# Illumina/strelka

Measured on AMD Instinct MI355X. Metric: candidate-alignment scoring cells/s (read bases x candidate alignments; Strelka2 has no pair-HMM, SURVEY.md section 0) + germline loci/s + 40x WGS-like germline wall-clock (e2e) + 110x/40x somatic wall-clock (e2e_somatic), higher is better.
Workload: dtype f64; 1 GPU; germline chr20-style synthetic (BASELINE.json configs[1]).  Headline: scoreCandidateAlignment as one function -- per GPU per step 65536 reads of 150 bp x 87.9 candidate alignments each (5-7 candidate indels around them), from the candidate alignments the device search left (PCal) to one double each: one kernel (F5: the walk of each alignment's path + the terms of its bases, penalties and clips).  ; read_len=150

## Files before the change

include/strelka_amd.h:

```cpp
#ifndef STRELKA_AMD_H
#define STRELKA_AMD_H

#include <stddef.h>
#include <stdint.h>

#ifdef __cplusplus
extern "C" {
#endif

#define SK_VERSION 100


int sk_device_count(void);
void* sk_host_alloc(size_t bytes);
void sk_host_free(void* p);
int sk_init(int device);
int sk_init_strict(int device);
void sk_shutdown(void);
const char* sk_last_error(void);
int sk_version(void);
int sk_is_initialized(void);
int sk_sync_mode(void);
int sk_libm_restated(void);

int sk_broker_client(void);
int sk_broker_enable(int on);
int sk_broker_serve(int device, const char* socket_name, int idle_seconds);
int sk_broker_selftest(int n, uint32_t mul);

int sk_check_device_errors(void);

int sk_debug_set_g3_variant(int variant);
int sk_debug_g3_global_pass_count(void);
int sk_debug_force_device_libm(int on);
void sk_debug_grown_bytes(int64_t* device_bytes, int64_t* pinned_bytes);
void sk_debug_region_alleles(int no_edge_deletion, int ids_twice);
int sk_debug_f5_tail_order(const int32_t* cal_off, int32_t n_reads, int32_t waves, int32_t shift, int32_t* first, int32_t* n, int32_t* order_out);
int64_t sk_debug_f5_tail_launches(void);

int sk_get_qscore_tables(double* q2p, double* q2lncompe, double* q2lne);


enum { SK_BAM_REF = 0, SK_BAM_A = 1, SK_BAM_C = 2, SK_BAM_G = 4, SK_BAM_T = 8, SK_BAM_ANY = 15 };

enum {
    SK_OP_BASES = 0,
    SK_OP_SOFT_CLIP = 1,
    SK_OP_NOBASE = 2
};
enum { SK_OPFLAG_NONCANDIDATE_PENALTY = 1 };

typedef struct sk_score_op {
    uint16_t length;
// ... 886 lines not shown
```

strelka_amd/capi.py:

```python
import ctypes as C
import os

import numpy as np

_HERE = os.path.dirname(os.path.abspath(__file__))
LIB_PATH = os.path.join(_HERE, "lib", "libstrelka_amd.so")

c_void_p = C.c_void_p


class ScoreOp(C.Structure):
    _fields_ = [("length", C.c_uint16), ("kind", C.c_uint8), ("flags", C.c_uint8), ("src", C.c_int32)]


SCORE_OP_DTYPE = np.dtype([("length", "<u2"), ("kind", "u1"), ("flags", "u1"), ("src", "<i4")])
OP_BASES, OP_SOFT_CLIP, OP_NOBASE = 0, 1, 2
OPFLAG_PENALTY = 1


class AlignBatch(C.Structure):
    _fields_ = [("n_reads", C.c_int32), ("n_cals", C.c_int32), ("n_ops", C.c_int64),
                ("read_off", c_void_p), ("read_code", c_void_p), ("read_qual", c_void_p),
                ("hap_off", c_void_p), ("hap_code", c_void_p), ("cal_off", c_void_p), ("op_off", c_void_p),
                ("ops", c_void_p), ("max_read_len", C.c_int32), ("max_hap_len", C.c_int32),
# ... 200 lines not shown
    "sk_intake_options_default", "sk_read_intake_obs_bound", "sk_read_intake", "sk_read_intake_dev", "sk_read_intake_scratch_bytes",
    "sk_ar_state_initial", "sk_ref_anchors", "sk_ref_anchors_dev", "sk_active_regions_bound", "sk_active_regions", "sk_active_regions_dev",
    "sk_sync_state_initial", "sk_sync_regions_bound", "sk_sync_active_regions", "sk_sync_active_regions_dev", "sk_sync_region_params", "sk_sync_region_params_dev",
    "sk_region_haplotypes_params", "sk_region_haplotypes_params_dev",
    "sk_region_haplotypes_seq_bound", "sk_region_haplotypes_support_bound", "sk_region_haplotypes_scratch_bytes", "sk_region_haplotypes", "sk_region_haplotypes_dev",
    "sk_region_alleles_allele_bound", "sk_region_alleles_insert_bound", "sk_region_alleles_scratch_bytes", "sk_region_alleles", "sk_region_alleles_dev", "sk_debug_region_alleles",
    "sk_align_builder_create", "sk_align_builder_destroy", "sk_align_builder_clear", "sk_align_builder_append", "sk_align_builder_add_read",
    "sk_align_builder_finish", "sk_align_builder_error", "sk_align_builder_set_host_threads",
    "sk_align_scores_default", "sk_global_align",
    "sk_pileup_options_default", "sk_pileup_reads", "sk_pileup_reads_dev", "sk_pileup_scratch_bytes",
    "sk_pileup_stream_create", "sk_pileup_stream_destroy", "sk_pileup_stream_begin_region", "sk_pileup_stream_push", "sk_pileup_stream_push_begin", "sk_pileup_stream_push_finish", "sk_pileup_stream_enable_evs_words", "sk_gvcf_site_summaries", "sk_gvcf_site_summaries_dev", "sk_gvcf_plain_runs_dev", "sk_gvcf_plain_runs", "sk_pileup_stream_set_gvcf_block_options",
    "sk_somatic_pileup_stream_create", "sk_somatic_pileup_stream_destroy", "sk_somatic_pileup_stream_begin_region", "sk_somatic_pileup_stream_push", "sk_somatic_pileup_stream_push_begin", "sk_somatic_pileup_stream_push_finish",
    "sk_realign_options_default", "sk_realign_job_create", "sk_realign_job_destroy", "sk_realign_job_error",
    "sk_realign_job_set_reference", "sk_realign_job_set_indels", "sk_realign_job_add_read", "sk_realign_job_add_reads", "sk_realign_job_get_batch",
    "sk_realign_job_finish", "sk_realign_job_run", "sk_realign_job_n_reads", "sk_realign_job_read_result",
    "sk_realign_job_clear_reads", "sk_realign_job_rescore", "sk_realign_job_indels_consulted", "sk_realign_job_enumeration_counts", "sk_realign_device_job_counts", "sk_debug_f5_tail_order", "sk_debug_f5_tail_launches", "sk_realign_reference_reads_outside", "sk_realign_job_stage3_counts", "sk_make_start_pos_alignment", "sk_get_end_pin_start_pos",
    "sk_germline_options_default", "sk_dependent_eprob", "sk_dependent_eprob_dev", "sk_site_digt_call",
    "sk_site_digt_call_dev", "sk_site_digt_call_fused", "sk_site_digt_call_fused_dev",
    "sk_somatic_snv_options_default", "sk_somatic_snv_call_batch", "sk_somatic_snv_call_batch_dev",
    "sk_somatic_snv_call_tiers", "sk_somatic_snv_call_tiers_dev", "sk_somatic_snv_tiers_scratch_bytes",
    "sk_indel_options_default", "sk_somatic_indel_options_default", "sk_indel_grid_lhood", "sk_indel_grid_lhood_dev",
    "sk_somatic_indel_call_batch", "sk_somatic_indel_call_tiers", "sk_allele_group_genotype_lhoods", "sk_allele_group_genotype_lhoods_dev",
    "sk_allele_group_genotype_lhoods_wide", "sk_allele_group_genotype_lhoods_wide_dev",
    "sk_allele_group_genotype_lhoods_xwide", "sk_allele_group_genotype_lhoods_xwide_dev",
    "sk_discover_indels_and_mismatches", "sk_global_align_scratch_bytes", "sk_global_align_dev", "sk_bai_query", "sk_bam_region_filter", "sk_gvcf_block_sites", "sk_gvcf_block_sites_dev",
]

_lib = None


def lib():
# ... 24 lines not shown
        L.sk_pileup_reads.argtypes = [C.POINTER(ReadBatchStruct), C.POINTER(PileupOptions), C.c_int, C.POINTER(PileupColumns)]
        L.sk_pileup_scratch_bytes.restype = C.c_int64
        L.sk_pileup_scratch_bytes.argtypes = [C.c_int32, C.c_int64, C.c_int32]
        L.sk_pileup_reads_dev.argtypes = [C.POINTER(ReadBatchStruct), C.c_int64, C.POINTER(PileupOptions), C.c_int,
                                          C.POINTER(PileupColumns), c_void_p, c_void_p]
        L.sk_realign_options_default.argtypes = [C.POINTER(RealignOptions)]
        L.sk_realign_job_create.restype = c_void_p
        L.sk_realign_job_create.argtypes = [C.POINTER(RealignOptions)]
        L.sk_realign_job_destroy.argtypes = [c_void_p]
        L.sk_realign_job_enumeration_counts.argtypes = [c_void_p, c_void_p, c_void_p, c_void_p]
        L.sk_realign_device_job_counts.argtypes = [c_void_p, c_void_p, c_void_p]
        L.sk_realign_device_job_counts.restype = None
        L.sk_debug_f5_tail_order.argtypes = [c_void_p, C.c_int32, C.c_int32, C.c_int32, c_void_p, c_void_p, c_void_p]
        L.sk_debug_f5_tail_launches.argtypes = []
        L.sk_debug_f5_tail_launches.restype = C.c_int64
        L.sk_realign_reference_reads_outside.argtypes = []
        L.sk_realign_reference_reads_outside.restype = C.c_int64
        L.sk_realign_job_stage3_counts.argtypes = [c_void_p, c_void_p, c_void_p]
        L.sk_realign_job_indels_consulted.argtypes = [c_void_p, c_void_p, C.c_int32]
        L.sk_realign_job_error.restype = C.c_char_p
        L.sk_realign_job_error.argtypes = [c_void_p]
        L.sk_realign_job_set_reference.argtypes = [c_void_p, C.c_char_p, C.c_int32, C.c_int32]
        L.sk_realign_job_set_indels.argtypes = [c_void_p, C.POINTER(IndelInfo), C.c_int32]
        L.sk_realign_job_add_read.argtypes = [c_void_p, C.POINTER(ReadInput)]
        L.sk_realign_job_add_reads.argtypes = [c_void_p, C.POINTER(ReadInput), C.c_int32]
        L.sk_realign_job_get_batch.argtypes = [c_void_p, C.POINTER(AlignBatch)]
        L.sk_realign_job_finish.argtypes = [c_void_p, c_void_p]
        L.sk_realign_job_run.argtypes = [c_void_p]
        L.sk_realign_job_n_reads.argtypes = [c_void_p]
        L.sk_realign_job_read_result.argtypes = [c_void_p, C.c_int32, C.POINTER(ReadResult)]
# ... 706 lines not shown
        a, b, c = C.c_int64(), C.c_int64(), C.c_int64()
        lib().sk_realign_job_enumeration_counts(self._j, C.byref(a), C.byref(b), C.byref(c))
        return a.value, b.value, c.value

    @staticmethod
    def device_job_counts():
        a, b, c = C.c_int64(), C.c_int64(), C.c_int64()
        lib().sk_realign_device_job_counts(C.byref(a), C.byref(b), C.byref(c))
        return a.value, b.value, c.value

    @staticmethod
    def f5_tail_launches():
        return int(lib().sk_debug_f5_tail_launches())

    @staticmethod
    def f5_tail_order(cal_off, waves, shift):
        cal_off = np.ascontiguousarray(cal_off, np.int32)
        n_reads = len(cal_off) - 1
        first, n = C.c_int32(-1), C.c_int32(-1)
        order = np.full(max(n_reads, 1), -2, np.int32)
        if lib().sk_debug_f5_tail_order(_p(cal_off), n_reads, int(waves), int(shift), C.byref(first), C.byref(n), _p(order)):
            raise StrelkaAmdError(last_error())
        return first.value, order[:n.value].copy()

    def stage3_counts(self):
        a, b = C.c_int64(), C.c_int64()
        lib().sk_realign_job_stage3_counts(self._j, C.byref(a), C.byref(b))
        return a.value, b.value

    def clear_reads(self):
# ... 798 lines not shown
```

strelka_amd/csrc/read_enumerate.hip:

```cpp

#include "sk_common.h"

#include "align_entry.h"
#include "read_enumerate.h"

#include <algorithm>
#include <chrono>
#include <climits>
#include <cstdio>
#include <cstdlib>
#include <cstring>
#include <vector>

using namespace skcore;

int sk_score_alignments_launch_hostleg(const sk_align_batch* b, double* dev_out_lnp, void* hip_stream);

namespace
{

static_assert(sizeof(PFrame) % 4 == 0 && sizeof(PCal) % 4 == 0, "frames move through LDS as 32-bit words");


struct EnumArgs
// ... 235 lines not shown
    a.sorted[a.cal_off[r] + rank] = a.grouped[g];
    }
}


enum { DYN_N_GROUPED = 0, DYN_N_CALS, DYN_N_LIGHT, DYN_N_HEAVY, DYN_FLAGS, DYN_MAX_CALS, DYN_REF_OUTSIDE, DYN_COUNT = 8 };
enum { DYNF_DEEPER = 1,
       DYNF_POOL_FULL = 2 };
enum { SEARCH_LEVELS = Caps::K + 2,
       CNT_LEVELS = 0,
       CNT_LEAVES = Caps::K + 3,
       CNT_NODES = (Caps::K + 5) & ~1,
       CNT_UNHANDLED = Caps::K + 7,
       CNT_DYN = Caps::K + 8,
       CNT_QUEUE = CNT_DYN + DYN_COUNT,
       N_COUNTERS = CNT_QUEUE + 2 };
static_assert(CNT_LEVELS + SEARCH_LEVELS + 1 == CNT_LEAVES && CNT_NODES > CNT_LEAVES && CNT_NODES + 2 <= CNT_UNHANDLED, "the counters' slots overlap");

template <typename V>
__device__ inline V block_exclusive_scan(const V v, V* wave_sums , V* total)
{
    const int lane = threadIdx.x & 63, wave = threadIdx.x >> 6, n_waves = blockDim.x >> 6;
    V x = v;
    for (int d = 1; d < 64; d <<= 1) {
        const V y = __shfl_up(x, d);
        if (lane >= d) x += y;
    }
    __syncthreads();
    if (lane == 63) wave_sums[wave] = x;
    __syncthreads();
    if (threadIdx.x == 0) {
// ... 468 lines not shown
static_assert(F5_TAB <= 32, "the table copy is a lane an entry, the consulted mask a bit an entry");

struct FusedScoreArgs
{
    FlatArgs f;
    const uint8_t* read_qual;
    const SkTables* tab;
    double* scores;
    unsigned* err;
    int32_t* n_unhandled;
    int32_t write_cals;
    unsigned long long* dbg;
    unsigned* queue;
    const int32_t* tail_order;
    uint32_t tail_first, tail_n;
};

constexpr int F5_SEGS = 16, F5_INDELS = 8;
constexpr int F5_STAMPS = 10;
constexpr int F5_SLOT = (F5_SEGS + 1) | 1;
__device__ __forceinline__ int f5_ent_word(const int k) { return k; }
constexpr int F5_ROW = 3;

struct F5Tab
{
    int32_t pos;
    uint32_t del, ins_len;
    uint32_t type_cand;
    int32_t ins_at;
};

template <int MAXR>
struct F5Lds
{
    uint8_t read[MAXR + 12];
    uint8_t hap[F5_MAX_POOL + 12];
    double row[(MAXR + 8) * F5_ROW];
    uint32_t slot[64 * F5_SLOT];
    F5Tab tab[F5_TAB];
};
constexpr int F5_Q_TERMS = 2 * (SK_NQ + 1);
constexpr size_t f5_block_granules(const size_t lds_object, const int waves)
{
    return (lds_object * size_t(waves) + 8 * size_t(F5_Q_TERMS) + 1279) / 1280;
}
static_assert(sizeof(F5Lds<152>) <= 10240 && 2 * f5_block_granules(sizeof(F5Lds<152>), 8) <= 128, "two eight-wave blocks of the short-read form to a CU");
static_assert(3 * f5_block_granules(sizeof(F5Lds<F5_MAX_READ>), 4) <= 128, "three four-wave blocks of the long-read form to a CU");
static_assert((152 + 12) % 4 == 0 && (F5_MAX_READ + 12) % 4 == 0 && (F5_MAX_POOL + 12) % 4 == 0, "the byte arrays' words stay aligned");
static_assert(INS_CAP <= 64, "a lane an insert");
static_assert(F5_CODE_PAD >= F5_MAX_POOL + 16 && F5_CODE_PAD % 4 == 0, "a window that leaves the reference stays inside the pad");

struct F5Rec
{
    uint32_t w0, w1, w2;
    uint64_t types;
    uint64_t l0, l1, l2, l3;
    uint64_t ind;
    int ind_lo;
    __device__ __forceinline__ int32_t pos() const { return int32_t(w0); }
// ... 212 lines not shown
    uint4 q0, q1, q2, q3, q4;
    uint32_t i0, i1, i2, i3;
};
__device__ __forceinline__ F5Raw f5_load_raw(const PCal* src)
{
    F5Raw w;
    const uint4* s4 = reinterpret_cast<const uint4*>(src);
    w.q0 = s4[0], w.q1 = s4[1], w.q2 = s4[2], w.q3 = s4[3], w.q4 = s4[4];
    const uint32_t* si = reinterpret_cast<const uint32_t*>(src->indels);
    w.i0 = si[0], w.i1 = si[1], w.i2 = si[2], w.i3 = si[3];
    return w;
}

constexpr int F5_INS_REG = 4;

template <int MAXR, bool TIMING>
__device__ __forceinline__ void f5_read(const FusedScoreArgs& fa, const int r, F5Lds<MAXR>& S, const double* const q_terms,
                                        const unsigned long long draw_cycles)
{
    auto now = [&]() -> unsigned long long { return TIMING ? (unsigned long long)clock64() : 0ull; };
    const FlatArgs& a = fa.f;
    int lane_of_read = threadIdx.x & 63;
    __asm__ volatile("" : "+v"(lane_of_read));
    const int lane = lane_of_read;
    unsigned long long stamp[F5_STAMPS];
    stamp[0] = now();
    const unsigned long long wall0 = TIMING ? (unsigned long long)wall_clock64() : 0ull;
    int g1_c0 = a.cal_off[r], g1_c1 = a.cal_off[r + 1];
    int32_t g1_status = a.status[r];
    int64_t g1_ro = a.read_off[r], g1_ro1 = a.read_off[r + 1];
    int32_t g1_P = a.hap_len[r], g1_win_begin = a.win_begin[r], g1_n_ins = a.n_ins[r], g1_win_len = a.win_len[r];
    __asm__ volatile("" : "+v"(g1_c0), "+v"(g1_c1), "+v"(g1_status), "+v"(g1_ro), "+v"(g1_ro1), "+v"(g1_P), "+v"(g1_win_begin), "+v"(g1_n_ins), "+v"(g1_win_len));
    auto uniform64 = [](const int64_t v) -> int64_t {
        return int64_t(uint64_t(uint32_t(__builtin_amdgcn_readfirstlane(int(uint32_t(uint64_t(v)))))) |
                       (uint64_t(uint32_t(__builtin_amdgcn_readfirstlane(int(uint32_t(uint64_t(v) >> 32))))) << 32));
    };
    const int c0 = __builtin_amdgcn_readfirstlane(g1_c0), c1 = __builtin_amdgcn_readfirstlane(g1_c1);
    const int32_t status_r = __builtin_amdgcn_readfirstlane(g1_status);
    const int64_t ro = uniform64(g1_ro), ro1 = uniform64(g1_ro1);
    const int32_t P = __builtin_amdgcn_readfirstlane(g1_P);
    const int32_t win_begin = __builtin_amdgcn_readfirstlane(g1_win_begin);
    const int n_ins = __builtin_amdgcn_readfirstlane(g1_n_ins);
    const int32_t win_len = __builtin_amdgcn_readfirstlane(g1_win_len);
    const double ln_quarter = fa.tab->ln_quarter, ln_noncand = fa.tab->ln_noncand;
    const int ncr = c1 - c0;
    if (ncr == 0 || status_r != ST_OK) return;
    for (int i = 1; i < F5_STAMPS; ++i) stamp[i] = 0;
    const int32_t L = int32_t(ro1 - ro);
    if (L > MAXR || P > F5_MAX_POOL) {
        if (lane == 0) atomicAdd(fa.n_unhandled, 1);
        return;
    }
    const int job_n_tab = a.job.n_tab;
    const bool whole_tab = job_n_tab <= F5_TAB;
    uint8_t* const order = S.hap + ((P + 8 + 3) & ~3);
    const bool sorted_order = (F5_SORT != 0) && ncr > 64 && ncr <= 256 && ((P + 8 + 3) & ~3) + ncr <= int(sizeof(S.hap));
    int32_t slot_next = 0;
    if (!sorted_order && lane < ncr) slot_next = a.list[c0 + lane];
    int32_t lst[4];
#pragma unroll
    for (int k = 0; k < 4; ++k) {
        lst[k] = 0;
        if (sorted_order && lane + 64 * k < ncr) lst[k] = a.list[c0 + lane + 64 * k];
    }
    F5Tab g;
    g.pos = 0, g.del = 0, g.ins_len = 0, g.type_cand = 0, g.ins_at = -1;
// ... 90 lines not shown
    }
    const bool ins_in_regs = n_ins <= F5_INS_REG && !__any(my_ins_len > 64);
    uint32_t ib[F5_INS_REG];
    int32_t ib_n[F5_INS_REG];
    uint32_t ib_src[F5_INS_REG];
#pragma unroll
    for (int k = 0; k < F5_INS_REG; ++k) {
        ib_n[k] = ins_in_regs ? __builtin_amdgcn_readlane(my_ins_len, k) : 0;
        ib_src[k] = uint32_t(__builtin_amdgcn_readlane(int(my_ins_src), k));
    }
#pragma unroll
    for (int k = 0; k < F5_INS_REG; ++k) {
        ib[k] = SK_BAM_ANY;
        if (lane < ib_n[k]) ib[k] = a.ins_code[ib_src[k] + uint32_t(lane)];
    }
    F5Raw raw0 = f5_load_raw(a.pool + slot_next);
    if (a.ref_outside && lane == 0) {
        const int64_t b = max(int64_t(win_begin), int64_t(a.ref_offset));
        const int64_t e = min(int64_t(win_begin) + int64_t(win_len), int64_t(a.ref_offset) + int64_t(a.ref_len));
        const int32_t outside = win_len - int32_t(max(e - b, int64_t(0)));
        if (outside > 0) atomicAdd(a.ref_outside, outside);
    }
    {
        uint32_t* const hap_w = reinterpret_cast<uint32_t*>(S.hap);
        const int n_words = (P + 8 + 3) >> 2;
#pragma unroll
        for (int k = 0; k < HAP_K; ++k) {
            const int w = lane + 64 * k;
            const int keep = win_len - 4 * w;
            const uint32_t m = (keep >= 4) ? 0xffffffffu : (keep <= 0) ? 0u : ((1u << (8 * keep)) - 1u);
            if (w < n_words) hap_w[w] = (hw[k] & m) | (ANY4 & ~m);
// ... 30 lines not shown
            if (q > 70u) {
                atomicOr(fa.err, unsigned(SK_DEVERR_QSCORE));
                q = 70u;
            }
            S.read[i] = code & 15u;
            if (i < L + 8) {
                const unsigned c = code & 15u;
                const bool adds = i < L && c != 15u;
                const double agree = adds ? q_terms[q] : 0.0;
                S.row[F5_ROW * i] = agree;
                S.row[F5_ROW * i + 1] = 0.0;
                S.row[F5_ROW * i + 2] = !adds ? 0.0 : (c == 0u) ? agree : q_terms[SK_NQ + 1 + q];
            }
        }
    }

    for (int j0 = 0; j0 < ncr; j0 += 64) {
        const int nc = min(64, ncr - j0);
        f5_wave_sync();
        const unsigned long long ta = now();
        if (j0 == 0) stamp[1] = ta;
        const bool has = lane < nc;
        uint32_t* const myslot = S.slot + lane * F5_SLOT;
        bool fits = true;
        const int my_j = has ? (sorted_order ? int(order[j0 + lane]) : j0 + lane) : 0;
        F5Rec rec;
        rec.w0 = rec.w1 = rec.w2 = 0;
        rec.types = 0;
        rec.l0 = rec.l1 = rec.l2 = rec.l3 = 0;
        rec.ind = 0;
        rec.ind_lo = 0;
        uint64_t ind_raw0 = 0, ind_raw1 = 0;
        if (j0 > 0) raw0 = f5_load_raw(a.pool + slot_next);
        if (has) {
            const F5Raw w = raw0;
            const uint4 q0 = w.q0, q1 = w.q1, q2 = w.q2, q3 = w.q3, q4 = w.q4;
            ind_raw0 = uint64_t(w.i0) | (uint64_t(w.i1) << 32);
            ind_raw1 = uint64_t(w.i2) | (uint64_t(w.i3) << 32);
            rec.w0 = q0.x;
            rec.w1 = q0.y;
            rec.w2 = q0.z;
            const unsigned nseg = (q0.z >> 8) & 0xffu, nind = (q0.z >> 16) & 0xffu;
            fits = (nseg <= unsigned(F5_SEGS) && nind <= unsigned(F5_INDELS));
            uint64_t types = 0;
            bool odd_type = false;
            auto pack4 = [&](const uint32_t a0, const uint32_t a1, const uint32_t a2, const uint32_t a3, const int first) -> uint64_t {
                types |= (uint64_t(a0 & 15u) | (uint64_t(a1 & 15u) << 4) | (uint64_t(a2 & 15u) << 8) | (uint64_t(a3 & 15u) << 12)) << (4 * first);
                odd_type = odd_type || (unsigned(first) < nseg && (a0 & 0xffffu) > 15u) || (unsigned(first + 1) < nseg && (a1 & 0xffffu) > 15u) ||
// ... 7 lines not shown
            rec.types = types;
            fits = fits && !odd_type;
        }
        auto raw_indel = [&](const int k) -> int { return int(int16_t(((k & 4) ? ind_raw1 : ind_raw0) >> (16 * (k & 3)))); };
        int tab_lo = 0;
        if (whole_tab) {
            bool out_of_table = false;
            if (has && fits) {
                auto check = [&](const int i) { out_of_table = out_of_table || i < 0 || i >= job_n_tab; };
                const int ni = rec.n_indels();
                for (int i = 0; i < ni; ++i) check(raw_indel(i));
                if (rec.lead() >= 0) check(rec.lead());
                if (rec.trail() >= 0) check(rec.trail());
            }
            if (__any((has && !fits) || out_of_table)) {
                if (lane == 0) atomicAdd(fa.n_unhandled, 1);
                return;
            }
            uint64_t ind = 0;
#pragma unroll
            for (int k = 0; k < F5_INDELS; ++k) ind |= uint64_t(unsigned(raw_indel(k)) & 63u) << (6 * k);
            rec.ind = ind;
            rec.ind_lo = 0;
        } else {
            int lo = INT_MAX, hi = INT_MIN;
            if (has && fits) {
                auto add = [&](const int i) {
                    lo = min(lo, i);
                    hi = max(hi, i);
                };
                const int ni = rec.n_indels();
                for (int i = 0; i < ni; ++i) add(raw_indel(i));
                if (rec.lead() >= 0) add(rec.lead());
                if (rec.trail() >= 0) add(rec.trail());
            }
#pragma unroll
            for (int d = 32; d > 0; d >>= 1) {
                lo = min(lo, __shfl_xor(lo, d));
                hi = max(hi, __shfl_xor(hi, d));
            }
            const int n_tab = (lo <= hi) ? hi - lo + 1 : 0;
            if (__any(has && !fits) || (n_tab > 0 && lo < 0) || n_tab > F5_TAB) {
                if (lane == 0) atomicAdd(fa.n_unhandled, 1);
                return;
            }
            tab_lo = n_tab ? lo : 0;
            uint64_t ind = 0;
#pragma unroll
            for (int k = 0; k < F5_INDELS; ++k) ind |= uint64_t(unsigned(raw_indel(k) - tab_lo) & 63u) << (6 * k);
            rec.ind = ind;
            rec.ind_lo = tab_lo;
            if (lane < n_tab) {
                const PIndel& g = a.job.tab[tab_lo + lane];
                F5Tab e;
                e.pos = g.pos;
                e.del = g.del;
                e.ins_len = g.ins_len;
                e.type_cand = unsigned(g.type) | (unsigned(g.cand) << 8);
                e.ins_at = -1;
// ... 19 lines not shown
            if (has) {
                const int ni = rec.n_indels();
                for (int i = 0; i < ni; ++i) cons |= 1u << ((rec.indel(i) - tab_lo) & 31);
                if (rec.lead() >= 0) cons |= 1u << ((rec.lead() - tab_lo) & 31);
                if (rec.trail() >= 0) cons |= 1u << ((rec.trail() - tab_lo) & 31);
                if (bad) a.status[r] = ST_FAIL;
            }
            if (a.job.consulted) {
#pragma unroll
                for (int d = 32; d > 0; d >>= 1) cons |= uint32_t(__shfl_xor(int(cons), d));
                cons_mine = lane < 32 && ((cons >> lane) & 1u) != 0u;
                if (cons_mine) cons_seen = a.job.consulted[tab_lo + lane];
            }
            (void)tA1;
        }
        if (j0 + 64 + lane < ncr) slot_next = a.list[c0 + (sorted_order ? int(order[j0 + 64 + lane]) : j0 + 64 + lane)];
        __builtin_amdgcn_wave_barrier();
        const unsigned long long td = now();
        stamp[4] += td - tc;
        if (has && !bad) {
            const double lnp = f5_sum(S, myslot, n_ent, ln_noncand, ln_quarter);
            fa.scores[c0 + my_j] = lnp;
        }
        if (cons_mine && cons_seen == 0) a.job.consulted[tab_lo + lane] = 1;
        raw0.q0 = raw0.q1 = raw0.q2 = raw0.q3 = raw0.q4 = make_uint4(0, 0, 0, 0);
        raw0.i0 = raw0.i1 = raw0.i2 = raw0.i3 = 0;
        stamp[5] += now() - td;
    }
    if (TIMING && fa.dbg && lane == 0) {
        stamp[6] = now();
        stamp[3] = TIMING ? (unsigned long long)wall_clock64() - wall0 : 0ull;
        stamp[8] = draw_cycles;
        stamp[9] = wall0;
        for (int i = 0; i < F5_STAMPS; ++i) fa.dbg[size_t(r) * F5_STAMPS + i] = stamp[i];
    }
}

template <int MAXR, bool TIMING, int WAVES>
__global__ __launch_bounds__(64 * WAVES) __attribute__((amdgpu_waves_per_eu(4, 4))) void flatten_score_kernel(const FusedScoreArgs fa, const int n_reads)
{
    __shared__ __attribute__((aligned(16))) F5Lds<MAXR> S[WAVES];
    __shared__ double q_terms[F5_Q_TERMS];
    for (int i = threadIdx.x; i < F5_Q_TERMS; i += 64 * WAVES) q_terms[i] = (i <= SK_NQ) ? fa.tab->q2lncompe[i] : fa.tab->q2mis[i - (SK_NQ + 1)];
    __syncthreads();
    const int wave = threadIdx.x >> 6, lane = threadIdx.x & 63;
    const unsigned n_waves = gridDim.x * unsigned(WAVES);
    unsigned h = unsigned(__builtin_amdgcn_readfirstlane(int(blockIdx.x * unsigned(WAVES) + unsigned(wave))));
    unsigned long long draw_cycles = 0;
    while (h < unsigned(n_reads)) {
        unsigned r = h;
        if (h - fa.tail_first < fa.tail_n) r = unsigned(__builtin_amdgcn_readfirstlane(fa.tail_order[h - fa.tail_first]));
        f5_read<MAXR, TIMING>(fa, int(r), S[wave], q_terms, draw_cycles);
        f5_wave_sync();
        const unsigned long long t0 = TIMING ? (unsigned long long)clock64() : 0ull;
        unsigned d = 0;
        if (lane == 0) d = atomicAdd(&fa.queue[0], 1u);
        int drawn = __builtin_amdgcn_readfirstlane(int(d));
        if (TIMING) __asm__ volatile("" : "+s"(drawn));
        h = n_waves + unsigned(drawn);
        draw_cycles = TIMING ? (unsigned long long)clock64() - t0 : 0ull;
    }
    if (lane == 0) {
        __threadfence();
        if (atomicAdd(&fa.queue[1], 1u) == gridDim.x * unsigned(WAVES) - 1u) {
            fa.queue[0] = 0u;
            fa.queue[1] = 0u;
        }
    }
}

struct F5Grid
{
    int wpb, blocks;
    int waves() const { return wpb * blocks; }
};
// ... 685 lines not shown
    if (!g_cals_gathered) {
        if (bufs().cals.reserve(sizeof(PCal) * size_t(g_n_cals))) return 1;
        SK_LAUNCH(gather_cals_kernel, dim3((g_n_cals + 63) / 64), dim3(64), 0, ctx.stream, g_cals_pool, g_cals_list, g_n_cals, bufs().cals.as<PCal>());
        SK_HIP(skrt::getLastError());
        g_cals_gathered = true;
    }
    SK_HIP(skrt::memcpyAsync(dst, bufs().cals.as<PCal>() + first, sizeof(PCal) * size_t(count), hipMemcpyDeviceToHost, ctx.stream));
    SK_HIP(skrt::streamSynchronize(ctx.stream));
    return 0;
}

namespace
{
int64_t g_jobs_one_wait = 0, g_jobs_one_wait_redone = 0, g_jobs_staged = 0;
int64_t g_tail_launches = 0;
struct JobSeconds
{
    double setup = 0, submit = 0, wait = 0, after = 0;
    ~JobSeconds()
    {
        if (std::getenv("SK_ENUM_JOB_SECONDS"))
            std::fprintf(stderr, "strelka_amd enum job seconds: jobs=%lld setup=%.4f submit=%.4f wait=%.4f after=%.4f\n", (long long)g_jobs_one_wait, setup, submit,
                         wait, after);
    }
} g_job_seconds;
}
extern "C" void sk_enum_device_job_counts(int64_t* one_wait, int64_t* one_wait_redone, int64_t* staged)
{
    if (one_wait) *one_wait = g_jobs_one_wait;
    if (one_wait_redone) *one_wait_redone = g_jobs_one_wait_redone;
// ... 21 lines not shown
        SK_HIP(skrt::malloc_(&d_order, 4 * size_t(T)));
        SK_HIP(skrt::memcpyAsync(d_off, cal_off, 4 * (size_t(n_reads) + 1), hipMemcpyHostToDevice, st));
        SK_HIP(skrt::memsetAsync(d_order, 0xff, 4 * size_t(T), st));
        launch_tail_order(st, TailArgs{ d_off, n_reads - T, T, shift, d_order });
        SK_HIP(skrt::getLastError());
        SK_HIP(skrt::memcpyAsync(order_out, d_order, 4 * size_t(T), hipMemcpyDeviceToHost, st));
        SK_HIP(skrt::streamSynchronize(st));
        return 0;
    };
    rc = run();
    if (d_off) (void)skrt::free_(d_off);
    if (d_order) (void)skrt::free_(d_order);
    return rc;
}
extern "C" int64_t sk_debug_f5_tail_launches(void) { return g_tail_launches; }

namespace
{
struct JobPlan
{
    const SkEnumInput* in = nullptr;
    EnumBuffers& B = bufs();
    hipStream_t st = nullptr;
    bool one_wait = false, with_stage3 = false;
    int n = 0;
    int64_t n_bases = 0, frame_cap = 0, pool_cap = 0;
    int W = 0;
    int max_order = 0;
    size_t in_bytes = 0, zero_bytes = 0, minmax_bytes = 0, mask_bytes = 0;
    size_t minmax_split = 0;
// ... 308 lines not shown
FusedScoreArgs fused_args(const JobPlan& p, const FlatArgs& fa)
{
    EnumBuffers& B = p.B;
    FusedScoreArgs fs;
    fs.f = fa;
    fs.read_qual = B.read_qual.as<uint8_t>();
    fs.tab = sk_ctx().dev_tables;
    fs.scores = B.scores.as<double>();
    fs.err = sk_ctx().dev_error_flags;
    fs.n_unhandled = B.counters.as<int32_t>() + CNT_UNHANDLED;
    fs.queue = B.counters.as<unsigned>() + CNT_QUEUE;
    fs.write_cals = 0;
    fs.dbg = nullptr;
    fs.tail_order = nullptr;
    fs.tail_first = fs.tail_n = 0;
    return fs;
}

void plan_tail(const JobPlan& p, FusedScoreArgs& fs)
{
    EnumBuffers& B = p.B;
    const int W = f5_grid(p.n, fs.f.max_read_len).waves();
    const int shift = f5_tail_shift(W), T = f5_tail_window(p.n, W, shift);
    if (T == 0) return;
    launch_tail_order(p.st, TailArgs{ fs.f.cal_off, p.n - T, T, shift, B.tail_order.as<int32_t>() });
    ++g_tail_launches;
    fs.tail_order = B.tail_order.as<int32_t>();
    fs.tail_first = uint32_t(p.n - T);
    fs.tail_n = uint32_t(T);
}
// ... 152 lines not shown
        SK_LAUNCH(job_stage_out_kernel, dim3(blocks), dim3(256), 0, st, static_cast<const uint4*>(B.zero_arena.p), static_cast<uint4*>(B.h_zero_arena.p), n_a,
                  static_cast<const uint4*>(B.s3_out.p), static_cast<uint4*>(B.h_s3_out.p), n_b);
        SK_HIP(skrt::getLastError());
    } else {
        if (copy_down(st, B.h_zero_arena, B.zero_arena, p.zero_bytes) || copy_down(st, B.h_s3_out, B.s3_out, out_bytes)) return 1;
    }
    const auto t_submitted = std::chrono::steady_clock::now();
    SK_HIP(skrt::streamSynchronize(st));
    const auto t_waited = std::chrono::steady_clock::now();
    g_job_seconds.setup += std::chrono::duration<double>(t_setup - p.t_begin).count();
    g_job_seconds.submit += std::chrono::duration<double>(t_submitted - t_setup).count();
    g_job_seconds.wait += std::chrono::duration<double>(t_waited - t_submitted).count();
    p.lap("one sequence");
    const int32_t* h_counters = B.h_counters.as<int32_t>();
    const int32_t* const h_dyn = h_counters + CNT_DYN;
    if (h_dyn[DYN_FLAGS] != 0 || h_counters[CNT_UNHANDLED] > 0) {
        if (p.timing)
            std::fprintf(stderr, "[enum-dev] one sequence: flags %d, reads outside F5's form %d -> the staged chain\n", h_dyn[DYN_FLAGS], h_counters[CNT_UNHANDLED]);
        *redo = true;
        return 0;
    }
    ++g_jobs_one_wait;
    out->warn = narrow_warn(B, n);
    int32_t* h_cal_off = B.h_cal_off.as<int32_t>();
    std::memcpy(h_cal_off, B.h_cal_off_z.p, 4 * size_t(n + 1));
    const int32_t n_cals = h_cal_off[n];
    g_n_cals = n_cals;
    g_cals_pool = fa.pool;
    g_cals_list = fa.list;
    g_scores = B.scores.as<double>();
// ... 233 lines not shown
            g_cals_gathered = true;
            if (copy_down(st, B.h_cals, B.cals, sizeof(PCal) * size_t(n_cals))) return 1;
        }
        remember_fused(p, fs, n_cals);
        if (after_scores(p, out, fa, false)) return 1;
        if (fetch_zero(p, B.counters, B.counters, 4 * size_t(N_COUNTERS))) return 1;
        if (fetch_zero(p, B.status, B.status, 4 * size_t(n))) return 1;
        SK_HIP(skrt::streamSynchronize(st));
        chain = B.h_counters.as<int32_t>()[CNT_UNHANDLED] > 0;
    }
    if (chain && run_chain(p, out, fa)) return 1;
    if (fetch_zero(p, B.consulted, B.consulted, size_t(in->n_tab))) return 1;
    if (fetch_zero(p, B.counters, B.counters, 4 * size_t(N_COUNTERS))) return 1;
    SK_HIP(skrt::streamSynchronize(st));
    out->ref_reads_outside = B.h_counters.as<int32_t>()[CNT_DYN + DYN_REF_OUTSIDE];
    p.lap("done");
    return 0;
}
}

extern "C" int sk_enum_device_run(const SkEnumInput* in, SkEnumOutput* out)
{
    const bool enabled = !(std::getenv("SK_ENUM_ONE_WAIT") != nullptr && std::strcmp(std::getenv("SK_ENUM_ONE_WAIT"), "0") == 0);
    const bool fused_enabled = !(std::getenv("SK_A5_FUSED") != nullptr && std::strcmp(std::getenv("SK_A5_FUSED"), "0") == 0);
    if (enabled && fused_enabled && in && in->want_scores && in->want_stage3 && in->n_reads > 0 && in->n_reads <= ONE_WAIT_MAX_READS &&
        in->max_read_len <= F5_MAX_READ) {
        JobPlan p;
        bool redo = false;
        const int rc = start_job(in, out, true, p) || run_one_wait(p, out, &redo);
        if (rc != 0 || !redo) return rc;
// ... 1 lines not shown
    }
    JobPlan p;
    if (start_job(in, out, false, p)) return 1;
    return p.n == 0 ? 0 : run_staged(p, out);
}

static int f5_timing_report(hipStream_t st)
{
    FusedScoreArgs fs = g_last.fs;
    const size_t nb = size_t(g_last.n) * F5_STAMPS;
    SkDevBuf dbg;
    if (dbg.reserve(nb * 8)) return 1;
    unsigned long long* d = dbg.as<unsigned long long>();
    SK_HIP(skrt::memsetAsync(d, 0, nb * 8, st));
    fs.dbg = d;
    launch_flatten_score(g_last.n, st, fs);
    std::vector<unsigned long long> h(nb);
    SK_HIP(skrt::memcpyAsync(h.data(), d, nb * 8, hipMemcpyDeviceToHost, st));
    SK_HIP(skrt::streamSynchronize(st));
    dbg.drop();
    double sum[F5_STAMPS] = { 0 };
    unsigned long long first = ~0ull, last = 0;
    int nblk = 0, ndrawn = 0;
    for (int r = 0; r < g_last.n; ++r) {
        const unsigned long long* s = &h[size_t(r) * F5_STAMPS];
        if (s[6] == 0) continue;
        ++nblk;
        first = std::min(first, s[0]);
        last = std::max(last, s[6]);
        sum[0] += double(s[1] - s[0]);
        for (int i = 2; i <= 5; ++i) sum[i] += double(s[i]);
        sum[7] += double(s[7]);
        sum[6] += double(s[6] - s[0]);
        sum[8] += double(s[8]);
        ndrawn += s[8] != 0;
// ... 85 lines not shown
```

Before: 905.0 billion cells/s.

## Let idle waves help score other waves' 64-alignment rounds within a block

Splits the per-read F5 scoring into a prologue and per-64-alignment rounds. A wave publishes its read's descriptor and round counter in LDS, and waves whose queue has run dry claim rounds of a sibling's read by atomic increment. This is meant to cut the tail where one wave grinds through a read with many candidate alignments while the other waves in its block sit idle. In exchange it adds LDS per wave, atomics on every round, spin-sleep polling capped by wall clock, and extra list and pool loads for helper rounds. It is on by default and can be turned off with SK_F5_SHARE=0.

Result: faster. 917.1 billion cells/s (median of 6 runs) (+1.3%).

```diff
diff --git a/include/strelka_amd.h b/include/strelka_amd.h
--- a/include/strelka_amd.h
+++ b/include/strelka_amd.h
@@ -37,6 +37,8 @@
 void sk_debug_region_alleles(int no_edge_deletion, int ids_twice);
 int sk_debug_f5_tail_order(const int32_t* cal_off, int32_t n_reads, int32_t waves, int32_t shift, int32_t* first, int32_t* n, int32_t* order_out);
 int64_t sk_debug_f5_tail_launches(void);
+int64_t sk_debug_f5_shared_rounds(void);
+int64_t sk_debug_f5_late_turn_downs(void);
 
 int sk_get_qscore_tables(double* q2p, double* q2lncompe, double* q2lne);
 
diff --git a/strelka_amd/capi.py b/strelka_amd/capi.py
--- a/strelka_amd/capi.py
+++ b/strelka_amd/capi.py
@@ -238,7 +238,7 @@
     "sk_realign_options_default", "sk_realign_job_create", "sk_realign_job_destroy", "sk_realign_job_error",
     "sk_realign_job_set_reference", "sk_realign_job_set_indels", "sk_realign_job_add_read", "sk_realign_job_add_reads", "sk_realign_job_get_batch",
     "sk_realign_job_finish", "sk_realign_job_run", "sk_realign_job_n_reads", "sk_realign_job_read_result",
-    "sk_realign_job_clear_reads", "sk_realign_job_rescore", "sk_realign_job_indels_consulted", "sk_realign_job_enumeration_counts", "sk_realign_device_job_counts", "sk_debug_f5_tail_order", "sk_debug_f5_tail_launches", "sk_realign_reference_reads_outside", "sk_realign_job_stage3_counts", "sk_make_start_pos_alignment", "sk_get_end_pin_start_pos",
+    "sk_realign_job_clear_reads", "sk_realign_job_rescore", "sk_realign_job_indels_consulted", "sk_realign_job_enumeration_counts", "sk_realign_device_job_counts", "sk_debug_f5_tail_order", "sk_debug_f5_tail_launches", "sk_debug_f5_shared_rounds", "sk_debug_f5_late_turn_downs", "sk_realign_reference_reads_outside", "sk_realign_job_stage3_counts", "sk_make_start_pos_alignment", "sk_get_end_pin_start_pos",
     "sk_germline_options_default", "sk_dependent_eprob", "sk_dependent_eprob_dev", "sk_site_digt_call",
     "sk_site_digt_call_dev", "sk_site_digt_call_fused", "sk_site_digt_call_fused_dev",
     "sk_somatic_snv_options_default", "sk_somatic_snv_call_batch", "sk_somatic_snv_call_batch_dev",
@@ -293,6 +293,10 @@
         L.sk_debug_f5_tail_order.argtypes = [c_void_p, C.c_int32, C.c_int32, C.c_int32, c_void_p, c_void_p, c_void_p]
         L.sk_debug_f5_tail_launches.argtypes = []
         L.sk_debug_f5_tail_launches.restype = C.c_int64
+        L.sk_debug_f5_shared_rounds.argtypes = []
+        L.sk_debug_f5_shared_rounds.restype = C.c_int64
+        L.sk_debug_f5_late_turn_downs.argtypes = []
+        L.sk_debug_f5_late_turn_downs.restype = C.c_int64
         L.sk_realign_reference_reads_outside.argtypes = []
         L.sk_realign_reference_reads_outside.restype = C.c_int64
         L.sk_realign_job_stage3_counts.argtypes = [c_void_p, c_void_p, c_void_p]
@@ -1029,6 +1033,14 @@
         return int(lib().sk_debug_f5_tail_launches())
 
     @staticmethod
+    def f5_shared_rounds():
+        return int(lib().sk_debug_f5_shared_rounds())
+
+    @staticmethod
+    def f5_late_turn_downs():
+        return int(lib().sk_debug_f5_late_turn_downs())
+
+    @staticmethod
     def f5_tail_order(cal_off, waves, shift):
         cal_off = np.ascontiguousarray(cal_off, np.int32)
         n_reads = len(cal_off) - 1
diff --git a/strelka_amd/csrc/read_enumerate.hip b/strelka_amd/csrc/read_enumerate.hip
--- a/strelka_amd/csrc/read_enumerate.hip
+++ b/strelka_amd/csrc/read_enumerate.hip
@@ -273,7 +273,8 @@
        CNT_UNHANDLED = Caps::K + 7,
        CNT_DYN = Caps::K + 8,
        CNT_QUEUE = CNT_DYN + DYN_COUNT,
-       N_COUNTERS = CNT_QUEUE + 2 };
+       CNT_SHARED = CNT_QUEUE + 2,
+       N_COUNTERS = CNT_SHARED + 2 };
 static_assert(CNT_LEVELS + SEARCH_LEVELS + 1 == CNT_LEAVES && CNT_NODES > CNT_LEAVES && CNT_NODES + 2 <= CNT_UNHANDLED, "the counters' slots overlap");
 
 template <typename V>
@@ -772,10 +773,12 @@
     unsigned* queue;
     const int32_t* tail_order;
     uint32_t tail_first, tail_n;
+    int32_t share;
+    unsigned* shared_rounds;
 };
 
 constexpr int F5_SEGS = 16, F5_INDELS = 8;
-constexpr int F5_STAMPS = 10;
+constexpr int F5_STAMPS = 11;
 constexpr int F5_SLOT = (F5_SEGS + 1) | 1;
 __device__ __forceinline__ int f5_ent_word(const int k) { return k; }
 constexpr int F5_ROW = 3;
@@ -798,9 +801,10 @@
     F5Tab tab[F5_TAB];
 };
 constexpr int F5_Q_TERMS = 2 * (SK_NQ + 1);
+constexpr size_t F5_SHARE_BYTES = 36;
 constexpr size_t f5_block_granules(const size_t lds_object, const int waves)
 {
-    return (lds_object * size_t(waves) + 8 * size_t(F5_Q_TERMS) + 1279) / 1280;
+    return ((lds_object + F5_SHARE_BYTES) * size_t(waves) + 8 * size_t(F5_Q_TERMS) + 8 + 1279) / 1280;
 }
 static_assert(sizeof(F5Lds<152>) <= 10240 && 2 * f5_block_granules(sizeof(F5Lds<152>), 8) <= 128, "two eight-wave blocks of the short-read form to a CU");
 static_assert(3 * f5_block_granules(sizeof(F5Lds<F5_MAX_READ>), 4) <= 128, "three four-wave blocks of the long-read form to a CU");
@@ -1043,18 +1047,38 @@
 
 constexpr int F5_INS_REG = 4;
 
+struct F5Desc
+{
+    int32_t r, c0, ncr, L, P, win_begin, sorted_order;
+};
+struct F5Own
+{
+    int32_t slot_next;
+    F5Raw raw0;
+    int my_ins_idx;
+    int32_t my_ins_off;
+    unsigned long long stamp[F5_STAMPS], wall0;
+};
+struct F5Share
+{
+    uint32_t claim;
+    F5Desc d;
+    uint32_t dry_at;
+};
+static_assert(sizeof(F5Share) == F5_SHARE_BYTES, "f5_block_granules counts the claim words and descriptors");
+
 template <int MAXR, bool TIMING>
-__device__ __forceinline__ void f5_read(const FusedScoreArgs& fa, const int r, F5Lds<MAXR>& S, const double* const q_terms,
-                                        const unsigned long long draw_cycles)
+__device__ __forceinline__ bool f5_prologue(const FusedScoreArgs& fa, const int r, F5Lds<MAXR>& S, const double* const q_terms, F5Desc& desc,
+                                            F5Own& own)
 {
     auto now = [&]() -> unsigned long long { return TIMING ? (unsigned long long)clock64() : 0ull; };
     const FlatArgs& a = fa.f;
+    unsigned long long(&stamp)[F5_STAMPS] = own.stamp;
     int lane_of_read = threadIdx.x & 63;
     __asm__ volatile("" : "+v"(lane_of_read));
     const int lane = lane_of_read;
-    unsigned long long stamp[F5_STAMPS];
     stamp[0] = now();
-    const unsigned long long wall0 = TIMING ? (unsigned long long)wall_clock64() : 0ull;
+    own.wall0 = TIMING ? (unsigned long long)wall_clock64() : 0ull;
     int g1_c0 = a.cal_off[r], g1_c1 = a.cal_off[r + 1];
     int32_t g1_status = a.status[r];
     int64_t g1_ro = a.read_off[r], g1_ro1 = a.read_off[r + 1];
@@ -1071,14 +1095,13 @@
     const int32_t win_begin = __builtin_amdgcn_readfirstlane(g1_win_begin);
     const int n_ins = __builtin_amdgcn_readfirstlane(g1_n_ins);
     const int32_t win_len = __builtin_amdgcn_readfirstlane(g1_win_len);
-    const double ln_quarter = fa.tab->ln_quarter, ln_noncand = fa.tab->ln_noncand;
     const int ncr = c1 - c0;
-    if (ncr == 0 || status_r != ST_OK) return;
+    if (ncr == 0 || status_r != ST_OK) return false;
     for (int i = 1; i < F5_STAMPS; ++i) stamp[i] = 0;
     const int32_t L = int32_t(ro1 - ro);
     if (L > MAXR || P > F5_MAX_POOL) {
         if (lane == 0) atomicAdd(fa.n_unhandled, 1);
-        return;
+        return false;
     }
     const int job_n_tab = a.job.n_tab;
     const bool whole_tab = job_n_tab <= F5_TAB;
@@ -1199,7 +1222,7 @@
         ib[k] = SK_BAM_ANY;
         if (lane < ib_n[k]) ib[k] = a.ins_code[ib_src[k] + uint32_t(lane)];
     }
-    F5Raw raw0 = f5_load_raw(a.pool + slot_next);
+    own.raw0 = f5_load_raw(a.pool + slot_next);
     if (a.ref_outside && lane == 0) {
         const int64_t b = max(int64_t(win_begin), int64_t(a.ref_offset));
         const int64_t e = min(int64_t(win_begin) + int64_t(win_len), int64_t(a.ref_offset) + int64_t(a.ref_len));
@@ -1260,16 +1283,47 @@
             }
         }
     }
-
-    for (int j0 = 0; j0 < ncr; j0 += 64) {
+    desc.r = r, desc.c0 = c0, desc.ncr = ncr, desc.L = L, desc.P = P, desc.win_begin = win_begin, desc.sorted_order = sorted_order ? 1 : 0;
+    own.slot_next = slot_next;
+    own.my_ins_idx = my_ins_idx;
+    own.my_ins_off = my_ins_off;
+    return true;
+}
+
+template <typename LDS>
+__device__ __forceinline__ int f5_list_index(const LDS& D, const F5Desc& d, const int at)
+{
+    const uint8_t* const order = D.hap + ((d.P + 8 + 3) & ~3);
+    return d.c0 + (d.sorted_order ? int(order[at]) : at);
+}
+
+template <int MAXR, bool TIMING, typename NextRound>
+__device__ __forceinline__ bool f5_round(const FusedScoreArgs& fa, F5Lds<MAXR>& D, uint32_t* const slots, const F5Desc& d, const int j, const bool mine,
+                                         F5Own& own, NextRound next_j, int& j_next)
+{
+    auto now = [&]() -> unsigned long long { return TIMING ? (unsigned long long)clock64() : 0ull; };
+    const FlatArgs& a = fa.f;
+    unsigned long long(&stamp)[F5_STAMPS] = own.stamp;
+    F5Lds<MAXR>& S = D;
+    F5Raw& raw0 = own.raw0;
+    int32_t& slot_next = own.slot_next;
+    const int lane = threadIdx.x & 63;
+    const int r = d.r, c0 = d.c0, ncr = d.ncr, job_n_tab = a.job.n_tab;
+    const int32_t L = d.L, P = d.P, win_begin = d.win_begin;
+    const int my_ins_idx = own.my_ins_idx;
+    const int32_t my_ins_off = own.my_ins_off;
+    const double ln_quarter = fa.tab->ln_quarter, ln_noncand = fa.tab->ln_noncand;
+    {
+        const int j0 = 64 * j;
         const int nc = min(64, ncr - j0);
         f5_wave_sync();
         const unsigned long long ta = now();
-        if (j0 == 0) stamp[1] = ta;
+        if (mine && j0 == 0) stamp[1] = ta;
         const bool has = lane < nc;
-        uint32_t* const myslot = S.slot + lane * F5_SLOT;
+        uint32_t* const myslot = slots + lane * F5_SLOT;
+        const bool whole_tab = job_n_tab <= F5_TAB;
         bool fits = true;
-        const int my_j = has ? (sorted_order ? int(order[j0 + lane]) : j0 + lane) : 0;
+        const int my_j = has ? f5_list_index(S, d, j0 + lane) - c0 : 0;
         F5Rec rec;
         rec.w0 = rec.w1 = rec.w2 = 0;
         rec.types = 0;
@@ -1277,7 +1331,7 @@
         rec.ind = 0;
         rec.ind_lo = 0;
         uint64_t ind_raw0 = 0, ind_raw1 = 0;
-        if (j0 > 0) raw0 = f5_load_raw(a.pool + slot_next);
+        if (!mine || j0 > 0) raw0 = f5_load_raw(a.pool + slot_next);
         if (has) {
             const F5Raw w = raw0;
             const uint4 q0 = w.q0, q1 = w.q1, q2 = w.q2, q3 = w.q3, q4 = w.q4;
@@ -1315,8 +1369,11 @@
                 if (rec.trail() >= 0) check(rec.trail());
             }
             if (__any((has && !fits) || out_of_table)) {
-                if (lane == 0) atomicAdd(fa.n_unhandled, 1);
-                return;
+                if (lane == 0) {
+                    atomicAdd(fa.n_unhandled, 1);
+                    if (j > 0) atomicAdd(fa.shared_rounds + 1, 1u);
+                }
+                return false;
             }
             uint64_t ind = 0;
 #pragma unroll
@@ -1342,8 +1399,11 @@
             }
             const int n_tab = (lo <= hi) ? hi - lo + 1 : 0;
             if (__any(has && !fits) || (n_tab > 0 && lo < 0) || n_tab > F5_TAB) {
-                if (lane == 0) atomicAdd(fa.n_unhandled, 1);
-                return;
+                if (lane == 0) {
+                    atomicAdd(fa.n_unhandled, 1);
+                    if (j > 0) atomicAdd(fa.shared_rounds + 1, 1u);
+                }
+                return false;
             }
             tab_lo = n_tab ? lo : 0;
             uint64_t ind = 0;
@@ -1393,7 +1453,8 @@
             }
             (void)tA1;
         }
-        if (j0 + 64 + lane < ncr) slot_next = a.list[c0 + (sorted_order ? int(order[j0 + 64 + lane]) : j0 + 64 + lane)];
+        j_next = mine ? next_j() : -1;
+        if (j_next >= 0 && 64 * j_next + lane < ncr) slot_next = a.list[f5_list_index(S, d, 64 * j_next + lane)];
         __builtin_amdgcn_wave_barrier();
         const unsigned long long td = now();
         stamp[4] += td - tc;
@@ -1405,39 +1466,128 @@
         raw0.q0 = raw0.q1 = raw0.q2 = raw0.q3 = raw0.q4 = make_uint4(0, 0, 0, 0);
         raw0.i0 = raw0.i1 = raw0.i2 = raw0.i3 = 0;
         stamp[5] += now() - td;
-    }
-    if (TIMING && fa.dbg && lane == 0) {
-        stamp[6] = now();
-        stamp[3] = TIMING ? (unsigned long long)wall_clock64() - wall0 : 0ull;
+        if (mine) stamp[10] += 1;
+    }
+    return true;
+}
+
+template <bool TIMING>
+__device__ __forceinline__ void f5_store_stamps(const FusedScoreArgs& fa, const int r, F5Own& own, const unsigned long long draw_cycles)
+{
+    if (TIMING && fa.dbg && (threadIdx.x & 63) == 0) {
+        unsigned long long(&stamp)[F5_STAMPS] = own.stamp;
+        stamp[6] = (unsigned long long)clock64();
+        stamp[3] = (unsigned long long)wall_clock64() - own.wall0;
         stamp[8] = draw_cycles;
-        stamp[9] = wall0;
+        stamp[9] = own.wall0;
         for (int i = 0; i < F5_STAMPS; ++i) fa.dbg[size_t(r) * F5_STAMPS + i] = stamp[i];
     }
 }
 
+constexpr int F5_HELP_NAP = 64;
+constexpr unsigned F5_HELP_CAP = 2000000u;
 template <int MAXR, bool TIMING, int WAVES>
 __global__ __launch_bounds__(64 * WAVES) __attribute__((amdgpu_waves_per_eu(4, 4))) void flatten_score_kernel(const FusedScoreArgs fa, const int n_reads)
 {
     __shared__ __attribute__((aligned(16))) F5Lds<MAXR> S[WAVES];
     __shared__ double q_terms[F5_Q_TERMS];
+    __shared__ F5Share share[WAVES];
+    __shared__ unsigned busy;
     for (int i = threadIdx.x; i < F5_Q_TERMS; i += 64 * WAVES) q_terms[i] = (i <= SK_NQ) ? fa.tab->q2lncompe[i] : fa.tab->q2mis[i - (SK_NQ + 1)];
+    if (threadIdx.x < unsigned(WAVES)) share[threadIdx.x].claim = 0u, share[threadIdx.x].dry_at = 0u;
+    if (threadIdx.x == 0) busy = unsigned(WAVES);
     __syncthreads();
-    const int wave = threadIdx.x >> 6, lane = threadIdx.x & 63;
+    const int wave = __builtin_amdgcn_readfirstlane(int(threadIdx.x >> 6)), lane = threadIdx.x & 63;
     const unsigned n_waves = gridDim.x * unsigned(WAVES);
+    auto published = [&](const int ncr) -> bool { return WAVES > 1 && fa.share != 0 && fa.f.job.n_tab <= F5_TAB && ncr > 64 && ncr < (0x8000 << 6); };
     unsigned h = unsigned(__builtin_amdgcn_readfirstlane(int(blockIdx.x * unsigned(WAVES) + unsigned(wave))));
     unsigned long long draw_cycles = 0;
-    while (h < unsigned(n_reads)) {
-        unsigned r = h;
-        if (h - fa.tail_first < fa.tail_n) r = unsigned(__builtin_amdgcn_readfirstlane(fa.tail_order[h - fa.tail_first]));
-        f5_read<MAXR, TIMING>(fa, int(r), S[wave], q_terms, draw_cycles);
+    auto draw = [&]() {
         f5_wave_sync();
         const unsigned long long t0 = TIMING ? (unsigned long long)clock64() : 0ull;
-        unsigned d = 0;
-        if (lane == 0) d = atomicAdd(&fa.queue[0], 1u);
-        int drawn = __builtin_amdgcn_readfirstlane(int(d));
+        unsigned got = 0;
+        if (lane == 0) got = atomicAdd(&fa.queue[0], 1u);
+        int drawn = __builtin_amdgcn_readfirstlane(int(got));
         if (TIMING) __asm__ volatile("" : "+s"(drawn));
         h = n_waves + unsigned(drawn);
         draw_cycles = TIMING ? (unsigned long long)clock64() - t0 : 0ull;
+    };
+    F5Desc d;
+    F5Own own;
+    d.r = d.c0 = d.ncr = d.L = d.P = d.win_begin = d.sorted_order = 0;
+    int j = -1, src = wave;
+    for (;;) {
+        if (j < 0 && h < unsigned(n_reads)) {
+            unsigned r = h;
+            if (h - fa.tail_first < fa.tail_n) r = unsigned(__builtin_amdgcn_readfirstlane(fa.tail_order[h - fa.tail_first]));
+            if (!f5_prologue<MAXR, TIMING>(fa, int(r), S[wave], q_terms, d, own)) {
+                draw();
+                continue;
+            }
+            j = 0;
+            if (published(d.ncr)) {
+                __builtin_amdgcn_fence(__ATOMIC_RELEASE, "workgroup");
+                __builtin_amdgcn_wave_barrier();
+                if (lane == 0) {
+                    share[wave].d = d;
+                    __builtin_amdgcn_fence(__ATOMIC_RELEASE, "workgroup");
+                    __hip_atomic_store(&share[wave].claim, 1u | (unsigned((d.ncr + 63) >> 6) << 16), __ATOMIC_RELAXED, __HIP_MEMORY_SCOPE_WORKGROUP);
+                }
+            }
+        } else if (j < 0) {
+            unsigned dry_at = unsigned(__builtin_amdgcn_readfirstlane(int(share[wave].dry_at)));
+            if (dry_at == 0u) {
+                if (lane == 0) __hip_atomic_fetch_add(&busy, ~0u, __ATOMIC_RELAXED, __HIP_MEMORY_SCOPE_WORKGROUP);
+                if (!(WAVES > 1 && fa.share != 0)) break;
+                dry_at = unsigned(wall_clock64()) | 1u;
+                if (lane == 0) share[wave].dry_at = dry_at;
+            }
+            int look = threadIdx.x & 63;
+            __asm__ volatile("" : "+v"(look));
+            unsigned w = 0;
+            if (look < WAVES && look != wave) w = __hip_atomic_load(&share[look].claim, __ATOMIC_RELAXED, __HIP_MEMORY_SCOPE_WORKGROUP);
+            const unsigned long long open = __ballot((w & 0xffffu) < (w >> 16));
+            if (open == 0ull) {
+                const unsigned left = __hip_atomic_load(&busy, __ATOMIC_RELAXED, __HIP_MEMORY_SCOPE_WORKGROUP);
+                if (__builtin_amdgcn_readfirstlane(int(left)) == 0 || unsigned(wall_clock64()) - dry_at > F5_HELP_CAP) break;
+                __builtin_amdgcn_s_sleep(F5_HELP_NAP);
+                continue;
+            }
+            const int o = __builtin_amdgcn_readfirstlane(__builtin_ctzll(open));
+            unsigned old = 0;
+            if (lane == 0) old = __hip_atomic_fetch_add(&share[o].claim, 1u, __ATOMIC_RELAXED, __HIP_MEMORY_SCOPE_WORKGROUP);
+            old = unsigned(__builtin_amdgcn_readfirstlane(int(old)));
+            if ((old & 0xffffu) >= (old >> 16)) continue;
+            __builtin_amdgcn_fence(__ATOMIC_ACQUIRE, "workgroup");
+            const F5Desc& p = share[o].d;
+            d.r = __builtin_amdgcn_readfirstlane(p.r), d.c0 = __builtin_amdgcn_readfirstlane(p.c0), d.ncr = __builtin_amdgcn_readfirstlane(p.ncr);
+            d.L = __builtin_amdgcn_readfirstlane(p.L), d.P = __builtin_amdgcn_readfirstlane(p.P);
+            d.win_begin = __builtin_amdgcn_readfirstlane(p.win_begin), d.sorted_order = __builtin_amdgcn_readfirstlane(p.sorted_order);
+            j = int(old & 0xffffu), src = o;
+            own.slot_next = (64 * j + lane < d.ncr) ? fa.f.list[f5_list_index(S[src], d, 64 * j + lane)] : 0;
+            own.my_ins_idx = -1, own.my_ins_off = 0;
+        }
+        const bool mine = src == wave;
+        int j_next = -1;
+        const bool went = f5_round<MAXR, TIMING>(
+            fa, S[src], S[wave].slot, d, j, mine, own,
+            [&]() -> int {
+                int nj = j + 1;
+                if (published(d.ncr)) {
+                    unsigned old = 0;
+                    if (lane == 0) old = __hip_atomic_fetch_add(&share[wave].claim, 1u, __ATOMIC_RELAXED, __HIP_MEMORY_SCOPE_WORKGROUP);
+                    nj = __builtin_amdgcn_readfirstlane(int(old)) & 0xffff;
+                }
+                return 64 * nj < d.ncr ? nj : -1;
+            },
+            j_next);
+        if (!mine && went && lane == 0) atomicAdd(fa.shared_rounds, 1u);
+        j = (mine && went) ? j_next : -1;
+        if (mine && j < 0) {
+            if (went) f5_store_stamps<TIMING>(fa, d.r, own, draw_cycles);
+            else if (published(d.ncr) && lane == 0) __hip_atomic_store(&share[wave].claim, 0u, __ATOMIC_RELAXED, __HIP_MEMORY_SCOPE_WORKGROUP);
+            draw();
+        }
     }
     if (lane == 0) {
         __threadfence();
@@ -2153,6 +2303,8 @@
 {
 int64_t g_jobs_one_wait = 0, g_jobs_one_wait_redone = 0, g_jobs_staged = 0;
 int64_t g_tail_launches = 0;
+int64_t g_late_turn_downs = 0;
+int64_t g_shared_rounds = 0;
 struct JobSeconds
 {
     double setup = 0, submit = 0, wait = 0, after = 0;
@@ -2204,6 +2356,8 @@
     return rc;
 }
 extern "C" int64_t sk_debug_f5_tail_launches(void) { return g_tail_launches; }
+extern "C" int64_t sk_debug_f5_shared_rounds(void) { return g_shared_rounds; }
+extern "C" int64_t sk_debug_f5_late_turn_downs(void) { return g_late_turn_downs; }
 
 namespace
 {
@@ -2542,6 +2696,9 @@
     fs.dbg = nullptr;
     fs.tail_order = nullptr;
     fs.tail_first = fs.tail_n = 0;
+    static const bool share = [] { const char* e = std::getenv("SK_F5_SHARE"); return !(e && std::strcmp(e, "0") == 0); }();
+    fs.share = share ? 1 : 0;
+    fs.shared_rounds = B.counters.as<unsigned>() + CNT_SHARED;
     return fs;
 }
 
@@ -2724,6 +2881,8 @@
     p.lap("one sequence");
     const int32_t* h_counters = B.h_counters.as<int32_t>();
     const int32_t* const h_dyn = h_counters + CNT_DYN;
+    g_shared_rounds += h_counters[CNT_SHARED];
+    g_late_turn_downs += h_counters[CNT_SHARED + 1];
     if (h_dyn[DYN_FLAGS] != 0 || h_counters[CNT_UNHANDLED] > 0) {
         if (p.timing)
             std::fprintf(stderr, "[enum-dev] one sequence: flags %d, reads outside F5's form %d -> the staged chain\n", h_dyn[DYN_FLAGS], h_counters[CNT_UNHANDLED]);
@@ -2987,6 +3146,8 @@
     if (fetch_zero(p, B.counters, B.counters, 4 * size_t(N_COUNTERS))) return 1;
     SK_HIP(skrt::streamSynchronize(st));
     out->ref_reads_outside = B.h_counters.as<int32_t>()[CNT_DYN + DYN_REF_OUTSIDE];
+    g_shared_rounds += B.h_counters.as<int32_t>()[CNT_SHARED];
+    g_late_turn_downs += B.h_counters.as<int32_t>()[CNT_SHARED + 1];
     p.lap("done");
     return 0;
 }
@@ -3018,11 +3179,26 @@
     unsigned long long* d = dbg.as<unsigned long long>();
     SK_HIP(skrt::memsetAsync(d, 0, nb * 8, st));
     fs.dbg = d;
+    unsigned helped[2] = { 0, 0 };
+    SK_HIP(skrt::memcpyAsync(&helped[0], fs.shared_rounds, 4, hipMemcpyDeviceToHost, st));
     launch_flatten_score(g_last.n, st, fs);
+    SK_HIP(skrt::memcpyAsync(&helped[1], fs.shared_rounds, 4, hipMemcpyDeviceToHost, st));
     std::vector<unsigned long long> h(nb);
     SK_HIP(skrt::memcpyAsync(h.data(), d, nb * 8, hipMemcpyDeviceToHost, st));
     SK_HIP(skrt::streamSynchronize(st));
     dbg.drop();
+    {
+        const int32_t* const cal_off = bufs().h_cal_off.as<int32_t>();
+        long long by_owner = 0, implied = 0;
+        for (int r = 0; r < g_last.n; ++r) {
+            const unsigned long long* s = &h[size_t(r) * F5_STAMPS];
+            if (s[6] == 0) continue;
+            by_owner += (long long)s[10];
+            implied += (cal_off[r + 1] - cal_off[r] + 63) / 64;
+        }
+        std::fprintf(stderr, "[f5-timing] rounds: %lld scored by their owners + %u by helpers = %lld; cal_off implies %lld (sharing %s)\n", by_owner,
+                     helped[1] - helped[0], by_owner + (long long)(helped[1] - helped[0]), implied, fs.share ? "on" : "off");
+    }
     double sum[F5_STAMPS] = { 0 };
     unsigned long long first = ~0ull, last = 0;
     int nblk = 0, ndrawn = 0;
```
